# fpgasystems/gcow

Hardware: AMD Instinct MI355X
Metric: GiB/s device-resident fp32->ZFP encode, 256Mi-float bucket, 1/2/4/8 GPU (higher is better)
Workload: dtype f32; 1 GPU; c2_1d_fp32_fixed_rate16_256Mi_per_gpu; layout=1-D contiguous, 4-value blocks, mode=fixed-rate, minbits=64, maxbits=64, bucket_bytes_total=1073741824, launcher=none

## Files before the change

gcow_amd/csrc/enc_fixed1d.h:

```cpp
#pragma once

#include <hip/hip_runtime.h>
#include <stdint.h>

#include "codec_device.h"
#include "field_io.h"
#include "lean1d.h"

namespace gcow {

template <int DT>
__device__ __forceinline__ void load_block1d(const void* in, uint64_t nvals, uint32_t b, float* f)
{
  const uint64_t i0 = 4ull * b;
  if (i0 + 4 <= nvals) {
    load_row4<DT>(in, (int64_t)i0, f);
  } else {
    const uint32_t nv = (uint32_t)(nvals - i0);
#pragma unroll
    for (int x = 0; x < 4; x++) f[x] = load_elem<DT>(in, (int64_t)(i0 + pad_index(x, nv)));
  }
}

__device__ __forceinline__ uint32_t spread2_16(uint32_t x)
{
  x = (x | (x << 8)) & 0x00FF00FFu;
  x = (x | (x << 4)) & 0x0F0F0F0Fu;
  x = (x | (x << 2)) & 0x33333333u;
  x = (x | (x << 1)) & 0x55555555u;
  return x;
}

__device__ __forceinline__ uint64_t interleave4_16(uint32_t a, uint32_t b, uint32_t c, uint32_t d)
{
  const uint32_t P = spread2_16(a) | (spread2_16(c) << 1);
  const uint32_t Q = spread2_16(b) | (spread2_16(d) << 1);
  const uint32_t lo = spread2_16(P & 0xffffu) | (spread2_16(Q & 0xffffu) << 1);
  const uint32_t hi = spread2_16(P >> 16) | (spread2_16(Q >> 16) << 1);
  return (uint64_t)lo | ((uint64_t)hi << 32);
}

template <uint32_t WB>
__device__ __forceinline__ uint64_t encode_block1d_fixed(const float* f, const Params& p, const uint16_t* tab)
{
  float fa[4] = {f[0], f[1], f[2], f[3]};
  const int emax = block_emax<4>(fa);
  const uint32_t prec = precision(emax, p.maxprec, p.minexp, 1);
  if (!prec || emax == -127) return 0ull;
  const float s = cast_scale(emax);
  int32_t q[4];
#pragma unroll
  for (int i = 0; i < 4; i++) q[i] = cast1(fa[i], s);
  fwd_lift(q[0], q[1], q[2], q[3]);
  uint32_t u[4];
#pragma unroll
  for (int i = 0; i < 4; i++) u[i] = ((uint32_t)q[i] + 0xaaaaaaaau) ^ 0xaaaaaaaau;
  const int kmin = prec < 32 ? 32 - (int)prec : 0;
  uint64_t acc = 2ull * (uint32_t)(emax + 127) + 1ull;
  uint32_t pos = 9;
  {
    const int L0 = 31 - (int)__builtin_clz(u[0] | 1u) - (u[0] ? 0 : 1);
    const int L1 = 31 - (int)__builtin_clz(u[1] | 1u) - (u[1] ? 0 : 1);
    const int L2 = 31 - (int)__builtin_clz(u[2] | 1u) - (u[2] ? 0 : 1);
    const int L3 = 31 - (int)__builtin_clz(u[3] | 1u) - (u[3] ? 0 : 1);
    const int M0 = max(max(L0, L1), max(L2, L3));
    const int top = max(M0, kmin - 1);
    pos += (uint32_t)(31 - top);
    uint32_t n = 0;
    const int glo = max(L3, kmin);
    for (int k = top; k >= glo && pos < WB; --k) {
      const uint32_t x = ((u[0] >> k) & 1u) | (((u[1] >> k) & 1u) << 1) | (((u[2] >> k) & 1u) << 2) |
                         (((u[3] >> k) & 1u) << 3);
      const uint32_t e = tab[(n << 4) | x];
      acc |= (uint64_t)(e & 127u) << pos;
      pos += (e >> 7) & 7u;
      n = e >> 10;
    }
    const int kt = L3 - 1;
    if (pos < WB && kt >= kmin) {
      const uint32_t sh = (uint32_t)(31 - kt);
      const uint32_t g0 = __builtin_bitreverse32(u[0]) >> sh, g1 = __builtin_bitreverse32(u[1]) >> sh;
      const uint32_t g2 = __builtin_bitreverse32(u[2]) >> sh, g3 = __builtin_bitreverse32(u[3]) >> sh;
      uint64_t J = interleave4_16(g0 & 0xffffu, g1 & 0xffffu, g2 & 0xffffu, g3 & 0xffffu);
      const uint32_t cnt = (uint32_t)(kt - kmin + 1);
      if (cnt < 16) J &= (1ull << (4 * cnt)) - 1ull;
      acc |= J << pos;
    }
  }
  return WB == 64 ? acc : (acc & ((1ull << WB) - 1ull));
}

template <uint32_t WB, bool W2LOW = false>
__device__ __forceinline__ uint64_t encode_block1d_lean6(const float* f, const uint32_t* tab, const uint32_t* rs,
                                                         bool& special)
{
  uint32_t m;
  asm("v_max3_f32 %0, |%1|, |%2|, |%3|" : "=v"(m) : "v"(f[0]), "v"(f[1]), "v"(f[2]));
  asm("v_max_f32_e64 %0, %0, |%1|" : "+v"(m) : "v"(f[3]));
  special = m >= 0x7f800000u || __builtin_isunordered(f[0], f[1]) || __builtin_isunordered(f[2], f[3]);
  const uint32_t E = m >> 23;
  const float s = __uint_as_float((283u - E) << 23);
  uint32_t x = (uint32_t)cvt_i32_hw(f[0] * s), y = (uint32_t)cvt_i32_hw(f[1] * s);
  uint32_t z = (uint32_t)cvt_i32_hw(f[2] * s), w = (uint32_t)cvt_i32_hw(f[3] * s);
  auto asr = [](uint32_t v) { return (uint32_t)((int32_t)v >> 1); };
  constexpr uint32_t NB = 0xaaaaaaaau;
  x = asr(x + w); w -= x;
  z = asr(z + y); y -= z;
  x = asr(x + z); z -= x;
  w = asr(w + y); y -= w;
  const uint32_t u3 = (w + asr(y) + NB) ^ NB;
  const uint32_t u1 = (y - asr(w + asr(y)) + NB) ^ NB;
  const uint32_t u0 = (x + NB) ^ NB, u2 = (z + NB) ^ NB;
  const uint32_t o23 = u2 | u3;
  const uint32_t sh = __builtin_clz(u0 | u1 | o23 | 1u);
  const int M0 = 31 - (int)sh;
  const int jg = (int)min(ffbh_hw(o23), 31u) - (int)sh;
  const uint32_t w0 = u0 << sh, w1 = u1 << sh, w2 = u2 << sh, w3 = u3 << sh;
  const uint64_t Y = window_lds(rs, w0, w1, w2, w3);
  uint32_t pos = 9 + sh;
  uint32_t e = tab[(uint32_t)Y & 255u];
  uint32_t G = e >> 17, gl = (e >> 13) & 15u;
  int j = 4;
  e = tab5_next(tab, e, ((uint32_t)Y >> 8) & 255u);
  G |= (e >> 17) << gl;
  gl += (e >> 13) & 15u;
  const uint32_t hdr = m ? 2u * E + 3u : 0u;
  uint64_t acc = (uint64_t)hdr | ((uint64_t)G << pos);
  pos += gl;
#pragma unroll
  for (int jj = 4; jj < 16; jj += 2) {
    if (j < jj || !__any(jj <= jg)) break;
    e = tab5_next(tab, e, (uint32_t)(Y >> (4 * jj)) & 255u);
    const uint32_t code = pos < WB ? (e >> 17) : 0u;
    acc |= (uint64_t)code << pos;
    pos += (e >> 13) & 15u;
    j = jj + 2;
  }
  const bool tiny = m - 1u < (29u << 23) - 1u;
  special = special || (!tiny && jg >= 16 && pos < WB);
  if (j < 16 && pos < WB) acc |= (Y >> (4 * j)) << pos;
  const uint32_t p2 = pos + 4u * (uint32_t)(16 - j);
  if (__any(p2 < WB && M0 >= 16)) {
    uint64_t Y2;
    if constexpr (W2LOW) {
      Y2 = window_lds_low(rs, w0, w1, w2, w3);
    } else {
      const uint32_t s2 = sh + 16u;
      Y2 = window_lds(rs, u0 << s2, u1 << s2, u2 << s2, u3 << s2);
    }
    if (p2 < WB && M0 >= 16) acc |= Y2 << p2;
  }
  constexpr uint64_t TINY = tiny_payload_cx((int)WB - 9) << 9;
  acc = tiny ? (TINY | hdr) : acc;
  return WB == 64 ? acc : (acc & ((1ull << WB) - 1ull));
}

}
```

gcow_amd/csrc/enc_fixed1d.hip:

```cpp
#include <hip/hip_runtime.h>

#include <algorithm>
#include <stdint.h>

#include "codec_device.h"
#include "enc_fixed1d.h"
#include "field_io.h"
#include "kernels.h"
#include "lean1d.h"
#include "pipe.h"

#ifndef GCOW_C2_U
#define GCOW_C2_U 8
#endif

namespace gcow {

template <int DT, uint32_t WB, int U, uint32_t T = 256, int V = 0>
__global__ __launch_bounds__(T) void k_encode_fixed1d_np(const void* __restrict__ in, uint32_t nfull, Params p,
                                                         void* __restrict__ out)
{
  __shared__ __attribute__((aligned(16))) uint32_t tab[1280 + 1024];
  constexpr uint32_t IB = DT == DT_BF16 ? 8u : 16u;
  const pipe_v4i rin = buf_rsrc(in, nfull * IB), rout = buf_rsrc(out, nfull * (WB / 8));
  const uint32_t b0 = blockIdx.x * (T * U) + threadIdx.x;
  typename PipeRow<DT>::T r[U];
  if constexpr ((V & 1) != 0) {
    static_assert(T == 256, "table fill assumes 256 threads");
    constexpr int NT = 1280 / 256;
    const pipe_v4i rt = buf_rsrc(&g_plane_tab5, sizeof(PlaneTab2));
    uint32_t tv[NT];
#pragma unroll
    for (int i = 0; i < NT; i++) tv[i] = buf_load_u32((threadIdx.x + 256u * i) * 4u, rt);
#pragma unroll
    for (int k = 0; k < U; k++) r[k] = PipeRow<DT>::load((b0 + T * k) * IB, rin);
#pragma unroll
    for (uint32_t t = threadIdx.x; t < 1024; t += T) tab[1280 + t] = rspread_entry(t);
    asm volatile("s_waitcnt vmcnt(%5)" : "+v"(tv[0]), "+v"(tv[1]), "+v"(tv[2]), "+v"(tv[3]), "+v"(tv[4]) : "n"(U)
                 : "memory");
#pragma unroll
    for (int i = 0; i < NT; i++) tab[threadIdx.x + 256u * i] = tv[i];
  } else {
#pragma unroll
    for (int k = 0; k < U; k++) r[k] = PipeRow<DT>::load((b0 + T * k) * IB, rin);
#pragma unroll
    for (uint32_t t = threadIdx.x; t < 1280; t += T) tab[t] = g_plane_tab5.v[t];
#pragma unroll
    for (uint32_t t = threadIdx.x; t < 1024; t += T) tab[1280 + t] = rspread_entry(t);
  }
  __syncthreads();
#pragma unroll
  for (int k = 0; k < U; k++) {
    pipe_wait<U - 1>(r[k]);
    float f[4];
    PipeRow<DT>::unpack(r[k], f);
    bool special;
    uint64_t w = encode_block1d_lean6<WB, (V & 2) != 0>(f, tab, tab + 1280, special);
    if (special) {
      RegWriter64 rw{0ull, 0u};
      encode_block<1>(rw, f, p);
      w = WB == 64 ? rw.acc : (rw.acc & ((1ull << WB) - 1ull));
    }
    pipe_store<WB>((b0 + T * k) * (WB / 8), rout, w);
  }
}

template <int DT, uint32_t WB, int U>
__global__ __launch_bounds__(256) void k_copy_pattern1d(const void* __restrict__ in, uint32_t nfull,
                                                        void* __restrict__ out)
{
  constexpr uint32_t T = 256;
  constexpr uint32_t IB = DT == DT_BF16 ? 8u : 16u;
  const pipe_v4i rin = buf_rsrc(in, nfull * IB), rout = buf_rsrc(out, nfull * (WB / 8));
  const uint32_t b0 = blockIdx.x * (T * U) + threadIdx.x;
  typename PipeRow<DT>::T r[U];
#pragma unroll
  for (int k = 0; k < U; k++) r[k] = PipeRow<DT>::load((b0 + T * k) * IB, rin);
#pragma unroll
  for (int k = 0; k < U; k++) {
    pipe_wait<U - 1>(r[k]);
    float f[4];
    PipeRow<DT>::unpack(r[k], f);
    const uint64_t w = ((uint64_t)(__float_as_uint(f[0]) ^ __float_as_uint(f[1])) << 32) |
                       (__float_as_uint(f[2]) ^ __float_as_uint(f[3]));
    pipe_store<WB>((b0 + T * k) * (WB / 8), rout, w);
  }
}

template <int DT, uint32_t WB>
__global__ __launch_bounds__(256) void k_encode_fixed1d_generic(const void* __restrict__ in, uint32_t nfull, Params p,
                                                                void* __restrict__ out)
{
  __shared__ uint16_t tab[80];
  if (threadIdx.x < 80) tab[threadIdx.x] = plane_entry4(threadIdx.x);
  __syncthreads();
  constexpr int U = 2;
  const uint32_t b0 = blockIdx.x * (256u * U) + threadIdx.x;
  float f[U][4];
#pragma unroll
  for (int j = 0; j < U; j++) {
    const uint32_t b = b0 + 256u * j;
    if (b < nfull) load_row4<DT>(in, 4ll * b, f[j]);
  }
#pragma unroll
  for (int j = 0; j < U; j++) {
    const uint32_t b = b0 + 256u * j;
    if (b < nfull) {
      const uint64_t w = encode_block1d_fixed<WB>(f[j], p, tab);
      if constexpr (WB == 64) ((uint64_t*)out)[b] = w;
      else ((uint32_t*)out)[b] = (uint32_t)w;
    }
  }
}

template <int DT, uint32_t WB>
__global__ void k_encode_fixed1d_tail(const void* __restrict__ in, uint64_t nvals, uint32_t b, Params p,
                                      void* __restrict__ out)
{
  __shared__ uint16_t tab[80];
  if (threadIdx.x < 80) tab[threadIdx.x] = plane_entry4(threadIdx.x);
  __syncthreads();
  if (threadIdx.x) return;
  float f[4];
  load_block1d<DT>(in, nvals, b, f);
  const uint64_t w = encode_block1d_fixed<WB>(f, p, tab);
  if constexpr (WB == 64) ((uint64_t*)out)[b] = w;
  else ((uint32_t*)out)[b] = (uint32_t)w;
}

static inline hipStream_t S(void* s) { return (hipStream_t)s; }

template <int DT, uint32_t WB>
static void launch_fixed1d_t(const void* in, uint64_t nvals, const Params& p, void* out, hipStream_t st)
{
  const uint32_t nfull = (uint32_t)(nvals / 4);
  if (nfull) {
    const bool kmin0 = p.maxprec >= 32 && p.minexp <= -154;
    if (!kmin0) {
      k_encode_fixed1d_generic<DT, WB><<<(nfull + 511) / 512, 256, 0, st>>>(in, nfull, p, out);
    } else {
      constexpr uint32_t CH = 1u << 27;
      constexpr uint32_t IB = DT == DT_BF16 ? 8u : 16u;
      for (uint32_t c0 = 0; c0 < nfull; c0 += CH) {
        const uint32_t nc = min(CH, nfull - c0);
        const void* ic = (const char*)in + (size_t)c0 * IB;
        void* oc = (char*)out + (size_t)c0 * (WB / 8);
        constexpr int U = GCOW_C2_U;
        k_encode_fixed1d_np<DT, WB, U, 256, 3><<<(nc + 256 * U - 1) / (256 * U), 256, 0, st>>>(ic, nc, p, oc);
      }
    }
  }
  if (nvals % 4) k_encode_fixed1d_tail<DT, WB><<<1, 128, 0, st>>>(in, nvals, nfull, p, out);
}

hipError_t launch_copy_pattern1d(const void* in, int dtype, uint64_t nvals, uint32_t wb, void* out, void* stream)
{
  const uint32_t nfull = (uint32_t)(nvals / 4);
  constexpr uint32_t CH = 1u << 27;
  const uint32_t IB = dtype == DT_BF16 ? 8u : 16u;
  for (uint32_t c0 = 0; c0 < nfull; c0 += CH) {
    const uint32_t nc = std::min(CH, nfull - c0);
    const void* ic = (const char*)in + (size_t)c0 * IB;
    void* oc = (char*)out + (size_t)c0 * (wb / 8);
    const uint32_t g = (nc + 2047) / 2048;
    if (dtype == DT_BF16) {
      if (wb == 64) k_copy_pattern1d<DT_BF16, 64, 8><<<g, 256, 0, S(stream)>>>(ic, nc, oc);
      else k_copy_pattern1d<DT_BF16, 32, 8><<<g, 256, 0, S(stream)>>>(ic, nc, oc);
    } else {
      if (wb == 64) k_copy_pattern1d<DT_F32, 64, 8><<<g, 256, 0, S(stream)>>>(ic, nc, oc);
      else k_copy_pattern1d<DT_F32, 32, 8><<<g, 256, 0, S(stream)>>>(ic, nc, oc);
    }
  }
  return hipGetLastError();
}

hipError_t launch_encode_fixed1d(const void* in, int dtype, uint64_t nvals, uint32_t nblocks, const Params& p,
                                 void* out, void* stream)
{
  (void)nblocks;
  hipStream_t st = S(stream);
  if (dtype == DT_F32) {
    if (p.maxbits == 64) launch_fixed1d_t<DT_F32, 64>(in, nvals, p, out, st);
    else launch_fixed1d_t<DT_F32, 32>(in, nvals, p, out, st);
  } else {
    if (p.maxbits == 64) launch_fixed1d_t<DT_BF16, 64>(in, nvals, p, out, st);
    else launch_fixed1d_t<DT_BF16, 32>(in, nvals, p, out, st);
  }
  return hipGetLastError();
}

}
```

Before: 3888 GiB/s.

## Add straight-line fast-path encoder with wave-voted rare fallback for 1-D fixed-rate

Adds a branch-free fast encoder that handles the first two or three bit-plane pairs from the table, builds the rest directly from the interleaved window, and stores the result right away. Blocks flagged rare (NaN, unusual exponent range, late significant planes, short output) take a wave-voted slow path that finishes the plane loop and overwrites the store. Constants are pinned in scalar registers via inline asm, and the default variant selector now enables this path. Ablation hooks (nop padding, an out-of-line fallback) are also added behind macros. The aim is to cut per-block ALU work and divergence on the common case, at the cost of a possible second store and a more complex correctness surface.

```diff
diff --git a/gcow_amd/csrc/enc_fixed1d.h b/gcow_amd/csrc/enc_fixed1d.h
--- a/gcow_amd/csrc/enc_fixed1d.h
+++ b/gcow_amd/csrc/enc_fixed1d.h
@@ -155,4 +155,117 @@
   return WB == 64 ? acc : (acc & ((1ull << WB) - 1ull));
 }
 
-}
+
+
+struct StraightConsts {
+  uint32_t nb, row, emask, escale, elo, espan, jtop;
+};
+
+template <int NP>
+__device__ __forceinline__ StraightConsts straight_consts()
+{
+  StraightConsts K;
+  asm("s_mov_b32 %0, 0xaaaaaaaa" : "=s"(K.nb));
+  asm("s_mov_b32 %0, 0x1c00" : "=s"(K.row));
+  asm("s_mov_b32 %0, 0x7f800000" : "=s"(K.emask));
+  asm("s_mov_b32 %0, 0x8d800000" : "=s"(K.escale));
+  asm("s_mov_b32 %0, 0x0e800000" : "=s"(K.elo));
+  asm("s_mov_b32 %0, 0x71000000" : "=s"(K.espan));
+  asm("s_mov_b32 %0, %1" : "=s"(K.jtop) : "n"(1u << (32 - 2 * NP)));
+  return K;
+}
+
+struct StraightState {
+  uint64_t Y, acc;
+  uint32_t e, pos, sh, m, hdr, w0, w1, w2, w3;
+  bool nan;
+};
+
+template <uint32_t WB, int NP>
+__device__ __forceinline__ uint64_t encode_block1d_straight(const float* f, const uint32_t* tab, const uint32_t* rs,
+                                                            const StraightConsts& K, StraightState& S, bool& rare)
+{
+  static_assert(NP == 2 || NP == 3, "two or three plane pairs");
+  uint32_t m;
+  asm("v_max3_f32 %0, |%1|, |%2|, |%3|" : "=v"(m) : "v"(f[0]), "v"(f[1]), "v"(f[2]));
+  asm("v_max_f32_e64 %0, %0, |%1|" : "+v"(m) : "v"(f[3]));
+  const float s = __uint_as_float(K.escale - (m & K.emask));
+  uint32_t x = (uint32_t)cvt_i32_hw(f[0] * s), y = (uint32_t)cvt_i32_hw(f[1] * s);
+  uint32_t z = (uint32_t)cvt_i32_hw(f[2] * s), w = (uint32_t)cvt_i32_hw(f[3] * s);
+  auto asr = [](uint32_t v) { return (uint32_t)((int32_t)v >> 1); };
+  const uint32_t NB = K.nb;
+  x = asr(x + w); w -= x;
+  z = asr(z + y); y -= z;
+  x = asr(x + z); z -= x;
+  w = asr(w + y); y -= w;
+  const uint32_t u3 = (w + asr(y) + NB) ^ NB;
+  const uint32_t u1 = (y - asr(w + asr(y)) + NB) ^ NB;
+  const uint32_t u0 = (x + NB) ^ NB, u2 = (z + NB) ^ NB;
+  const uint32_t sh = __builtin_clz(u0 | u1 | u2 | u3 | 1u);
+  const uint32_t w0 = u0 << sh, w1 = u1 << sh, w2 = u2 << sh, w3 = u3 << sh;
+  const uint64_t Y = window_lds(rs, w0, w1, w2, w3);
+  uint32_t e = tab[(uint32_t)Y & 255u];
+  uint32_t G = e >> 17, gl = (e >> 13) & 15u;
+  e = *(const uint32_t*)((const char*)tab + ((e & K.row) | ((((uint32_t)Y >> 8) & 255u) << 2)));
+  G |= (e >> 17) << gl;
+  gl += (e >> 13) & 15u;
+  const bool nz = m != 0u;
+  uint32_t hdr;
+  asm("v_lshl_add_u32 %0, %1, 1, 3" : "=v"(hdr) : "v"(m >> 23));
+  hdr = nz ? hdr : 0u;
+  uint32_t pos = 9u + sh;
+  uint64_t acc = (uint64_t)hdr | ((uint64_t)G << pos);
+  pos += gl;
+  if constexpr (NP == 3) {
+    e = *(const uint32_t*)((const char*)tab + ((e & K.row) | ((((uint32_t)Y >> 16) & 255u) << 2)));
+    acc |= (uint64_t)(e >> 17) << pos;
+    pos += (e >> 13) & 15u;
+  }
+  const bool nan = (bool)__builtin_isunordered(f[0], f[1]) | (bool)__builtin_isunordered(f[2], f[3]);
+  const bool mag = m - K.elo >= K.espan, late = (w2 | w3) < K.jtop;
+  rare = nan | (nz & (mag | late));
+  if constexpr (WB == 64) rare = rare | (pos < 8u * NP);
+  S = StraightState{Y, acc, e, pos, sh, m, hdr, w0, w1, w2, w3, nan};
+  acc |= (Y >> (8 * NP)) << pos;
+  return WB == 64 ? acc : (acc & ((1ull << WB) - 1ull));
+}
+
+template <uint32_t WB, int NP, bool W2LOW>
+__device__ __forceinline__ uint64_t encode_block1d_rest(const StraightState& S, bool vote, const uint32_t* tab,
+                                                        const uint32_t* rs, bool& special)
+{
+  const uint32_t m = S.m, sh = S.sh;
+  const int M0 = 31 - (int)sh;
+  const int jg = (int)min(ffbh_hw(S.w2 | S.w3), 31u - sh);
+  const uint64_t Y = S.Y;
+  uint64_t acc = S.acc;
+  uint32_t e = S.e, pos = S.pos;
+  int j = 2 * NP;
+#pragma unroll
+  for (int jj = 2 * NP; jj < 16; jj += 2) {
+    if (j < jj || !__any(vote && jj <= jg)) break;
+    e = tab5_next(tab, e, (uint32_t)(Y >> (4 * jj)) & 255u);
+    const uint32_t code = pos < WB ? (e >> 17) : 0u;
+    acc |= (uint64_t)code << pos;
+    pos += (e >> 13) & 15u;
+    j = jj + 2;
+  }
+  const bool tiny = m - 1u < (29u << 23) - 1u;
+  special = m >= 0x7f800000u || S.nan || (!tiny && jg >= 16 && pos < WB);
+  if (j < 16 && pos < WB) acc |= (Y >> (4 * j)) << pos;
+  const uint32_t p2 = pos + 4u * (uint32_t)(16 - j);
+  if (__any(vote && p2 < WB && M0 >= 16)) {
+    uint64_t Y2;
+    if constexpr (W2LOW) {
+      Y2 = window_lds_low(rs, S.w0, S.w1, S.w2, S.w3);
+    } else {
+      Y2 = window_lds(rs, S.w0 << 16, S.w1 << 16, S.w2 << 16, S.w3 << 16);
+    }
+    if (p2 < WB && M0 >= 16) acc |= Y2 << p2;
+  }
+  constexpr uint64_t TINY = tiny_payload_cx((int)WB - 9) << 9;
+  acc = tiny ? (TINY | S.hdr) : acc;
+  return WB == 64 ? acc : (acc & ((1ull << WB) - 1ull));
+}
+
+}
diff --git a/gcow_amd/csrc/enc_fixed1d.hip b/gcow_amd/csrc/enc_fixed1d.hip
--- a/gcow_amd/csrc/enc_fixed1d.hip
+++ b/gcow_amd/csrc/enc_fixed1d.hip
@@ -13,8 +13,28 @@
 #ifndef GCOW_C2_U
 #define GCOW_C2_U 8
 #endif
+#ifndef GCOW_C2_V
+#define GCOW_C2_V 7
+#endif
+#ifndef GCOW_C2_NP
+#define GCOW_C2_NP 3
+#endif
+#ifndef GCOW_C2_ABL
+#define GCOW_C2_ABL 0
+#endif
 
 namespace gcow {
+
+#if GCOW_C2_ABL == 4
+template <uint32_t WB>
+__device__ __attribute__((noinline)) uint64_t encode_block1d_generic_ool(float f0, float f1, float f2, float f3, Params p)
+{
+  const float f[4] = {f0, f1, f2, f3};
+  RegWriter64 rw{0ull, 0u};
+  encode_block<1>(rw, f, p);
+  return WB == 64 ? rw.acc : (rw.acc & ((1ull << WB) - 1ull));
+}
+#endif
 
 template <int DT, uint32_t WB, int U, uint32_t T = 256, int V = 0>
 __global__ __launch_bounds__(T) void k_encode_fixed1d_np(const void* __restrict__ in, uint32_t nfull, Params p,
@@ -49,19 +69,61 @@
     for (uint32_t t = threadIdx.x; t < 1024; t += T) tab[1280 + t] = rspread_entry(t);
   }
   __syncthreads();
-#pragma unroll
-  for (int k = 0; k < U; k++) {
-    pipe_wait<U - 1>(r[k]);
-    float f[4];
-    PipeRow<DT>::unpack(r[k], f);
-    bool special;
-    uint64_t w = encode_block1d_lean6<WB, (V & 2) != 0>(f, tab, tab + 1280, special);
-    if (special) {
-      RegWriter64 rw{0ull, 0u};
-      encode_block<1>(rw, f, p);
-      w = WB == 64 ? rw.acc : (rw.acc & ((1ull << WB) - 1ull));
-    }
-    pipe_store<WB>((b0 + T * k) * (WB / 8), rout, w);
+  if constexpr ((V & 4) != 0) {
+    const StraightConsts K = straight_consts<GCOW_C2_NP>();
+#pragma unroll
+    for (int k = 0; k < U; k++) {
+      pipe_wait<U - 1>(r[k]);
+      float f[4];
+      PipeRow<DT>::unpack(r[k], f);
+      StraightState S;
+      bool rare;
+      const uint64_t w = encode_block1d_straight<WB, GCOW_C2_NP>(f, tab, tab + 1280, K, S, rare);
+      pipe_store<WB>((b0 + T * k) * (WB / 8), rout, w);
+      if (__any(rare)) {
+        bool special;
+        uint64_t w2 = encode_block1d_rest<WB, GCOW_C2_NP, (V & 2) != 0>(S, rare, tab, tab + 1280, special);
+        if (special) {
+          RegWriter64 rw{0ull, 0u};
+          encode_block<1>(rw, f, p);
+          w2 = WB == 64 ? rw.acc : (rw.acc & ((1ull << WB) - 1ull));
+        }
+        if (rare) pipe_store<WB>((b0 + T * k) * (WB / 8), rout, w2);
+      }
+    }
+  } else {
+#pragma unroll
+    for (int k = 0; k < U; k++) {
+      pipe_wait<U - 1>(r[k]);
+      float f[4];
+      PipeRow<DT>::unpack(r[k], f);
+#if GCOW_C2_ABL == 1
+      asm volatile("s_nop 0\n s_nop 0\n s_nop 0\n s_nop 0\n s_nop 0\n s_nop 0\n s_nop 0\n s_nop 0\n"
+                   "s_nop 0\n s_nop 0\n s_nop 0\n s_nop 0\n s_nop 0\n s_nop 0\n s_nop 0\n s_nop 0");
+#elif GCOW_C2_ABL == 2
+      {
+        uint32_t d0, d1, d2, d3;
+        asm volatile("v_xor_b32 %0, %4, %4\n v_xor_b32 %1, %5, %5\n v_xor_b32 %2, %6, %6\n v_xor_b32 %3, %7, %7\n"
+                     "v_xor_b32 %0, %5, %0\n v_xor_b32 %1, %6, %1\n v_xor_b32 %2, %7, %2\n v_xor_b32 %3, %4, %3\n"
+                     "v_xor_b32 %0, %6, %0\n v_xor_b32 %1, %7, %1\n v_xor_b32 %2, %4, %2\n v_xor_b32 %3, %5, %3\n"
+                     "v_xor_b32 %0, %7, %0\n v_xor_b32 %1, %4, %1\n v_xor_b32 %2, %5, %2\n v_xor_b32 %3, %6, %3"
+                     : "=&v"(d0), "=&v"(d1), "=&v"(d2), "=&v"(d3)
+                     : "v"(f[0]), "v"(f[1]), "v"(f[2]), "v"(f[3]));
+      }
+#endif
+      bool special;
+      uint64_t w = encode_block1d_lean6<WB, (V & 2) != 0>(f, tab, tab + 1280, special);
+      if (special) {
+#if GCOW_C2_ABL == 4
+        w = encode_block1d_generic_ool<WB>(f[0], f[1], f[2], f[3], p);
+#else
+        RegWriter64 rw{0ull, 0u};
+        encode_block<1>(rw, f, p);
+        w = WB == 64 ? rw.acc : (rw.acc & ((1ull << WB) - 1ull));
+#endif
+      }
+      pipe_store<WB>((b0 + T * k) * (WB / 8), rout, w);
+    }
   }
 }
 
@@ -146,7 +208,7 @@
         const void* ic = (const char*)in + (size_t)c0 * IB;
         void* oc = (char*)out + (size_t)c0 * (WB / 8);
         constexpr int U = GCOW_C2_U;
-        k_encode_fixed1d_np<DT, WB, U, 256, 3><<<(nc + 256 * U - 1) / (256 * U), 256, 0, st>>>(ic, nc, p, oc);
+        k_encode_fixed1d_np<DT, WB, U, 256, GCOW_C2_V><<<(nc + 256 * U - 1) / (256 * U), 256, 0, st>>>(ic, nc, p, oc);
       }
     }
   }
```

Result: no change. 3881 GiB/s (-0.2%).
